# Chthi/Ofighters

Measured on AMD Instinct MI355X. Metric: arena-steps/sec (env.step+obs+policy fwd) at 4096 arenas, 1/2/4/8 MI355X, higher is better.
Workload: dtype f32; 1 GPU; 4096 arenas x 8 ships per GPU, random-bot actions + step + 2D obs rasterise (u8 maps) + bi-head policy forward for 8 ship(s)/arena, trunk shared per arena (BASELINE configs[3]); arenas_per_gpu=4096, ships=8, laser_cap=512, episode_ticks=200, parallelism=arena-sharded x1, RCCL all-reduce of episodic scores only, laser_overflow=0, last_episode_score_sum=71103, last_episode_arenas=4096

## Files before the change

include/ofx.h:

```cpp
#ifndef OFX_H
#define OFX_H

#include <stddef.h>
#include <stdint.h>

#ifdef __cplusplus
extern "C" {
#endif

#define OFX_VERSION 1

enum {
  OFX_OK = 0,
  OFX_ERR_INVALID = -1,
  OFX_ERR_NO_DEVICE = -2,
  OFX_ERR_HIP = -3,
  OFX_ERR_STATE = -4,
  OFX_ERR_OVERFLOW = -5
};

typedef struct ofx_config {
  int32_t n_arenas;
  int32_t n_ships;
  int32_t laser_cap;
// ... 121 lines not shown
  int32_t n_tensors;
} ofx_policy_desc;
int ofx_policy_layout(const ofx_handle *h, ofx_policy_desc *desc_host);
int ofx_policy_forward(ofx_handle *h, const float *weights, const uint8_t *ship_mask,
                       float *act_values, int32_t *iaction, int32_t *ipointer,
                       float *heatmap);
int ofx_policy_pin_weights(ofx_handle *h, const float *weights);
#define OFX_OPT_TRUNK_PLAIN 1
#define OFX_OPT_FRAMES_REF  2
#define OFX_OPT_TRUNK_FUSE  4
#define OFX_OPT_BILINEAR_LEGACY 3
#define OFX_OPT_POLICY_BF16 5
#define OFX_OPT_FIT_PLAIN 6
#define OFX_OPT_TRUNK_SPARSE 7
int ofx_policy_trunk_stats(ofx_handle *h, int64_t *counts_host);
int ofx_set_option(ofx_handle *h, int32_t option, int32_t value);
int ofx_policy_explore(ofx_handle *h, double epsilon, uint64_t seed, uint32_t tick, int32_t collecting,
                       const uint8_t *ship_mask, int32_t *iaction, int32_t *ipointer);
int ofx_policy_actions(ofx_handle *h, const int32_t *iaction, const int32_t *ipointer,
                       const uint8_t *ship_mask, ofx_action *actions);

typedef struct ofx_transition {
  int32_t tick_prev, tick_next;
  int32_t frame_prev, frame_next;
  int32_t ship;
  int32_t iaction, px, py;
  int32_t reward;
  int32_t done;
  float head_prev[8], head_next[8];
} ofx_transition;
// ... 39 lines not shown
```

ofighters_amd/_native.py:

```python
import ctypes as C
import os

_HERE = os.path.dirname(os.path.abspath(__file__))
LIB_PATH = os.path.join(_HERE, "libofx.so")

OFX_OK = 0
OFX_ERR_INVALID = -1
OFX_ERR_NO_DEVICE = -2
OFX_ERR_HIP = -3
OFX_ERR_STATE = -4
OFX_ERR_OVERFLOW = -5

BOT_IDLE, BOT_RANDOM, BOT_TURRET, BOT_RUNNER, BOT_THRUST, BOT_SHOOT = range(6)
BEHAVIOURS = {None: BOT_IDLE, "idle": BOT_IDLE, "random": BOT_RANDOM, "turret": BOT_TURRET,
              "runner": BOT_RUNNER, "thrust": BOT_THRUST, "shoot": BOT_SHOOT}

(F_SHIP_X, F_SHIP_Y, F_SHIP_PX, F_SHIP_PY, F_SHIP_ALIVE, F_REWARD, F_SCORE, F_N_LASERS, F_LASER_X, F_LASER_Y,
 F_LASER_OWNER, F_LASER_DEAD, F_KILLER, F_TIME, F_LAST_SCORES, F_HULL, F_LASER_DX, F_LASER_DY,
 F_OBS_REWARD) = range(19)

MAP_U8, MAP_F32, MAP_F64, MAP_BITS = range(4)
OPT_TRUNK_PLAIN, OPT_FRAMES_REF, OPT_BILINEAR_LEGACY, OPT_TRUNK_FUSE, OPT_POLICY_BF16, OPT_FIT_PLAIN, OPT_TRUNK_SPARSE = 1, 2, 3, 4, 5, 6, 7


# ... 85 lines not shown
    "ofx_replay_capture": (_i, [_vp, _u32, _vp, _vp, _vp]),
    "ofx_agents_first_done": (_i, [_vp, _vp, _vp, C.POINTER(C.c_int32)]),
    "ofx_replay_count": (_i, [_vp, _vp, _vp]),
    "ofx_replay_rows_host": (_i, [_vp, C.c_int32, _vp, _vp]),
    "ofx_replay_frame_host": (_i, [_vp, C.c_int32, C.c_int32, _vp, _vp]),
    "ofx_replay_sample": (_i, [_vp, _u64, _u32, C.c_int32, _vp, _vp]),
    "ofx_replay_gather": (_i, [_vp, _vp, C.c_int32, _vp, _vp, _vp]),
    "ofx_replay_gather_valid": (_i, [_vp, _vp, _vp, C.c_int32, C.c_int32, C.c_int32, _vp, _vp, _vp, _vp]),
    "ofx_timer_start": (_i, [_vp]),
    "ofx_timer_stop": (_i, [_vp, C.POINTER(C.c_float)]),
    "ofx_event_record": (_i, [_vp, C.c_int32]),
    "ofx_policy_profile": (_i, [_vp, C.c_int32]),
    "ofx_policy_pin_weights": (_i, [_vp, _vp]),
    "ofx_set_option": (_i, [_vp, C.c_int32, C.c_int32]),
    "ofx_policy_trunk_stats": (_i, [_vp, C.POINTER(C.c_int64)]),
    "ofx_event_elapsed": (_i, [_vp, C.c_int32, C.c_int32, C.POINTER(C.c_float)]),
}

_LIB = None


def lib():
    global _LIB
    if _LIB is None:
        if not os.path.exists(LIB_PATH):
            raise ImportError(
                "ofighters_amd: %s is missing - build it with `make -C ofighters_amd/csrc` "
                "(there is no CPU fallback)" % LIB_PATH)
        L = C.CDLL(LIB_PATH)
        for name, (res, args) in SIGNATURES.items():
# ... 21 lines not shown
```

ofighters_amd/csrc/ofx_api.hip:

```cpp
#include <math.h>
#include <stdarg.h>
#include <stdlib.h>
#include <string.h>

#include <new>

#include "ofx_internal.h"

static thread_local char g_err[512] = "";

void ofx_set_error(const char *fmt, ...) {
  va_list ap;
  va_start(ap, fmt);
  vsnprintf(g_err, sizeof(g_err), fmt, ap);
  va_end(ap);
}

extern "C" const char *ofx_last_error(void) { return g_err; }
extern "C" int ofx_version(void) { return OFX_VERSION; }

extern "C" int ofx_device_count(void) {
  int n = 0;
  if (hipGetDeviceCount(&n) != hipSuccess) return 0;
  return n;
// ... 95 lines not shown
  h->cfg = *cfg;
  h->hit_thresh = sqrt_le_threshold((double)(cfg->laser_radius + cfg->ship_radius));
  const size_t NM = (size_t)cfg->n_arenas * cfg->n_ships, NL = (size_t)cfg->n_arenas * cfg->laser_cap,
               N = (size_t)cfg->n_arenas;
  ofx_state &s = h->st;
#define A(field, count) if ((rc = dev_alloc_zero(&s.field, count))) { ofx_destroy(h); return rc; }
  A(ship_x, NM) A(ship_y, NM) A(ship_px, NM) A(ship_py, NM) A(hull, NM)
  A(reward, NM) A(score, NM) A(obs_reward, NM) A(last_score, NM)
  A(alive, NM) A(killer, NM)
  A(time, N) A(n_lasers, N)
  A(laser_x, NL) A(laser_y, NL) A(laser_dx, NL) A(laser_dy, NL)
  A(laser_owner, NL) A(laser_dead, NL)
  A(overflow, 1) A(episode_sums, (size_t)cfg->n_ships + 1)
#undef A
  if ((rc = dev_alloc_zero(&h->bot_behaviours, (size_t)cfg->n_ships))) { ofx_destroy(h); return rc; }
  h->n_cus = 256;
  { int v = 0; if (hipDeviceGetAttribute(&v, hipDeviceAttributeMultiprocessorCount, cfg->device) == hipSuccess && v > 0) h->n_cus = v; }
  hipError_t e = hipStreamCreateWithFlags(&h->stream, hipStreamNonBlocking);
  if (e != hipSuccess) { ofx_set_error("hipStreamCreate: %s", hipGetErrorString(e)); ofx_destroy(h); return OFX_ERR_HIP; }
  h->own_stream = true;
  h->prof_base = -1;
  e = hipDeviceSynchronize();
  if (e != hipSuccess) { ofx_set_error("hipDeviceSynchronize: %s", hipGetErrorString(e)); ofx_destroy(h); return OFX_ERR_HIP; }
  *out = h;
  return OFX_OK;
}

extern "C" int ofx_destroy(ofx_handle *h) {
  if (!h) return OFX_OK;
  (void)hipSetDevice(h->cfg.device);
// ... 531 lines not shown
```

ofighters_amd/csrc/ofx_policy.hip:

```cpp
#include <stdlib.h>
#include <string.h>
#include <type_traits>
#include <utility>

#include "ofx_internal.h"
#include "ofx_head.h"
#include "ofx_diag.h"
#include "ofx_lowp.h"

#define PS 400

typedef float f32x4 __attribute__((ext_vector_type(4)));
typedef float f32x2 __attribute__((ext_vector_type(2)));
typedef float f32x16 __attribute__((ext_vector_type(16)));

static const int kTrunkCin[4] = {2, 8, 8, 8};
static const int kUpCin[4] = {1, 2, 4, 8};
static const int kUpCout[4] = {2, 4, 8, 1};

static int policy_layout(int32_t *offset, int32_t *count) {
  int n = 0, off = 0;
#define T(c) do { offset[n] = off; count[n] = (c); off += (c); n++; } while (0)
  for (int i = 0; i < 4; i++) { T(9 * kTrunkCin[i] * 8); T(8); T(8); T(8); T(8); T(8); }
  T(5008 * 100); T(100);
// ... 192 lines not shown

struct ConvParams {
  const float *in;
  const unsigned *bits[2];
  size_t bits_stride;
  const float *w, *b;
  float *out;
  const uint8_t *mask;
  const float *wbm;
  int H, W;
  int tiles_x, tiles;
  int legacy;
  int images;
  const int32_t *live;
  unsigned long long *stat;
};

template <int CIN, int COUT, int TH, int TW, int MODE, bool POOL, bool OUT_HWC>
__global__ __launch_bounds__(((TH / 2) * (TW / 2) + 63) / 64 * 64) void k_conv(ConvParams p) {
  constexpr int NT = (TH / 2) * (TW / 2);
  constexpr int NTB = (NT + 63) / 64 * 64;
  constexpr int TWP = TW + 2;
  __shared__ __align__(16) float tile[CIN][TH + 2][TWP];
  const int img = blockIdx.x / p.tiles, t = blockIdx.x - img * p.tiles;
  if (p.mask && !p.mask[img]) return;
  const int ty0 = (t / p.tiles_x) * TH, tx0 = (t % p.tiles_x) * TW;
  const int tid = threadIdx.x;
  const int H = p.H, W = p.W;

  constexpr int TOTAL = CIN * (TH + 2) * TWP;
// ... 470 lines not shown
          d0 = __builtin_amdgcn_mfma_f32_16x16x4f32(a0[aof(j)], bw[j], d0, 0, 0, 0);
          d1 = __builtin_amdgcn_mfma_f32_16x16x4f32(a1[aof(j)], bw[j], d1, 0, 0, 0);
        }
        finish(d0, T);
        finish(d1, T1);
      } else {
        f32x4 d0 = binit;
#pragma unroll
        for (int j = 0; j < NK; j++) d0 = __builtin_amdgcn_mfma_f32_16x16x4f32(a0[aof(j)], bw[j], d0, 0, 0, 0);
        finish(d0, T);
      }
    }
  }
}

template <int WD, int RP, int LS, int PLS, int LP>
__device__ __forceinline__ void ts_gemm_phase_sparse(const float *abase, const float (&bw)[LP ? 1 : 24], const lp_x4 (&bwb)[6],
                                                     const f32x4 binit, int wv, int lane,
                                                     int n16, int kq, int r, float *orow, const unsigned *nz, float k2,
                                                     bool top, bool bottom, unsigned &n_exec, unsigned &n_all,
                                                     unsigned long long *dbg = nullptr) {
#if OFX_TRUNK_STAMPS
  unsigned long long g_last = __builtin_amdgcn_s_memtime();
#define TSG_STAMP(i) do { const unsigned long long t_ = __builtin_amdgcn_s_memtime(); dbg[i] += t_ - g_last; g_last = t_; } while (0)
#else
#define TSG_STAMP(i) do { } while (0)
#endif
  constexpr int NK = 24, NPX = RP * WD, NT = (NPX + 15) / 16;
  auto aof = [&](int j) -> int { return (4 * (j & 1)) * PLS + ((j >> 1) / 3) * LS + ((j >> 1) % 3); };
  int toff[6];
#pragma unroll
  for (int J = 0; J < 6; J++) {
    const int tap = 2 * J + (kq >> 1);
    toff[J] = (4 * (kq & 1) - kq) * PLS + (tap / 3) * LS + tap % 3;
  }
  auto mm1 = [&](const float *a0, f32x4 &d0) {
    if constexpr (LP != 0) {
#pragma unroll
      for (int J = 0; J < 6; J++) {
        const float *q0 = a0 + toff[J];
        d0 = lp_mfma16<LP ? LP : 1>(lp_pk4<LP ? LP : 1>(q0[0], q0[PLS], q0[2 * PLS], q0[3 * PLS]), bwb[J], d0);
      }
    } else {
// ... 48 lines not shown
        any |= (rw[0] & m0) | (rw[1] & m1);
      }
      run = any != 0u;
    }
    run_mask = __builtin_amdgcn_ballot_w64(run);
  }
  auto store_const = [&](int T) {
    const int P = 16 * T + 4 * kq, rp = P / WD, x = P - rp * WD;
    if (r == 0) *reinterpret_cast<float2 *>(orow + rp * (WD / 2) + (x >> 1)) = make_float2(k2, k2);
  };
  auto run1 = [&](int T0) {
    f32x4 d0 = binit;
    mm1(a_of_tile(T0), d0);
    finish(d0, T0);
  };
#pragma unroll 1
  for (int T = wv; T < NT; T += 16)
    if (!((run_mask >> T) & 1ull)) store_const(T);
  if (wv == 0) { n_all += (unsigned)NT; n_exec += (unsigned)__builtin_popcountll(run_mask); }
  TSG_STAMP(0);
  unsigned long long m = run_mask;
  for (int i = 0; i < wv && m; i++) m &= m - 1;
#pragma unroll 1
  while (m) {
    const int T0 = __builtin_ctzll(m);
    unsigned long long m2 = m;
    for (int i = 0; i < 16 && m2; i++) m2 &= m2 - 1;
    if (m2) {
      const int T1 = __builtin_ctzll(m2);
      f32x4 d0 = binit, d1 = binit;
      mm2(a_of_tile(T0), a_of_tile(T1), d0, d1);
      finish(d0, T0);
      finish(d1, T1);
// ... 37 lines not shown
    const float *a0 = a_of_tile(T), *a1 = a_of_tile(two ? T1 : T);
    f32x4 d0 = binit, d1 = binit;
#pragma unroll
    for (int J = 0; J < 6; J++) {
      const float *q0 = a0 + toff[J], *q1 = a1 + toff[J];
      const lp_x4 A0 = lp_pk4<LP>(q0[0], q0[PLS], q0[2 * PLS], q0[3 * PLS]);
      const lp_x4 A1 = lp_pk4<LP>(q1[0], q1[PLS], q1[2 * PLS], q1[3 * PLS]);
      d0 = lp_mfma16<LP>(A0, bwb[J], d0);
      d1 = lp_mfma16<LP>(A1, bwb[J], d1);
    }
    finish(d0, T);
    if (two) finish(d1, T1);
  }
}

constexpr int F12_TH = 10, F12_LS = 216, F12_ROWS = F12_TH + 2;
constexpr int F12_PLS = (F12_ROWS * F12_LS + 63) / 64 * 64 + 16;
constexpr int F12_WR = 14, F12_BR = 2 * (F12_TH + 1) + 2;
constexpr int F12_THREADS = 1024;
static_assert(F12_PLS % 64 == 16 && F12_PLS % 4 == 0 && F12_LS % 4 == 0, "tile layout");
static_assert(2 * F12_BR * F12_WR <= F12_THREADS, "one staged word per thread");
static_assert((F12_TH + 1) * 100 <= 2 * F12_THREADS && F12_TH * 100 <= F12_THREADS, "pixel pairs per step");

template <int LP, bool SPARSE = false>
__global__ __launch_bounds__(F12_THREADS) void k_trunk12(ConvParams p, const float *lut) {
  constexpr bool BF16 = LP != 0;
  constexpr int W = PS, H = PS, H1 = PS / 2, H2 = PS / 4, LS = F12_LS, PLS = F12_PLS, NK = 24;
  __shared__ __align__(16) float slut[2 * 512 * 8];
  __shared__ __align__(16) float tile[8 * F12_PLS];
  __shared__ unsigned rows[2][2][F12_BR][F12_WR];
  __shared__ __align__(16) float halo[2][8][2][F12_LS];
  __shared__ unsigned nz[SPARSE ? 2 : 1][F12_ROWS][8];
  __shared__ __align__(16) float k1s[8], k2s[8];
  __shared__ float wbs[(SPARSE && !BF16) ? 24 * 64 : 1];
  unsigned n_exec = 0, n_all = 0, t_exec = 0, t_all = 0;
#if OFX_TRUNK_STAMPS
  unsigned long long st_a = 0, st_b = 0, st_last = __builtin_amdgcn_s_memtime(), st_begin = st_last, st_g[3] = {0, 0, 0};
#define T12_STAMP(acc) do { const unsigned long long t_ = __builtin_amdgcn_s_memtime(); acc += t_ - st_last; st_last = t_; } while (0)
#else
#define T12_STAMP(acc) do { } while (0)
#endif
  const int tid = threadIdx.x, lane = tid & 63;
  const int wv = __builtin_amdgcn_readfirstlane(tid >> 6);
  const int n16 = lane & 15, kq = lane >> 4, co = n16 >> 1, r = n16 & 1;

  auto bits_fetch = [&](int img, int pa, int pb) -> unsigned {
    const int nrows = 2 * (pb - pa) + 2;
    unsigned out = 0u;
    if (tid < 2 * nrows * F12_WR) {
// ... 16 lines not shown
  };
  auto bits_commit = [&](int buf, int pa, int pb, unsigned word) {
    const int nrows = 2 * (pb - pa) + 2;
    if (tid < 2 * nrows * F12_WR) {
      const int w = tid % F12_WR, rr = (tid / F12_WR) % nrows, ci = tid / (F12_WR * nrows);
      rows[buf][ci][rr][w] = word;
    }
  };

  for (int e = tid; e < 2 * 512 * 8 / 4; e += F12_THREADS)
    reinterpret_cast<f32x4 *>(slut)[e] = reinterpret_cast<const f32x4 *>(lut)[e];
  for (int e = tid; e < 8 * PLS / 4; e += F12_THREADS) reinterpret_cast<f32x4 *>(tile)[e] = f32x4{0.f, 0.f, 0.f, 0.f};
  for (int e = tid; e < 2 * 8 * 2 * LS / 4; e += F12_THREADS) reinterpret_cast<f32x4 *>(&halo[0][0][0][0])[e] = f32x4{0.f, 0.f, 0.f, 0.f};
  float bw[(BF16 || SPARSE) ? 1 : NK];
  lp_x4 bwb[6];
  if constexpr (BF16) ts_bw_lp<LP ? LP : 1>(p.wbm, n16, kq, bwb);
  else if constexpr (SPARSE) {
    for (int e = tid; e < NK * 64; e += F12_THREADS) wbs[e] = p.wbm[e];
  } else {
#pragma unroll
    for (int j = 0; j < NK; j++) bw[j] = p.wbm[j * 64 + lane];
  }
  const float bias = p.b[co];
  const f32x4 binit = {bias, bias, bias, bias};
  const float *abase = &tile[kq * PLS + 3];
  if constexpr (SPARSE) {
    __syncthreads();
    if (tid < 8) k1s[tid] = fmaxf(slut[tid] + slut[512 * 8 + tid], 0.f);
    for (int e = tid; e < 2 * F12_ROWS * 8; e += F12_THREADS) (&nz[0][0][0])[e] = 0u;
    __syncthreads();
    for (int e = tid; e < 8 * PLS; e += F12_THREADS) tile[e] = k1s[min(e / PLS, 7)];
    __syncthreads();
    if (wv == 0) {
      const float *a0 = abase + 2 * LS + 16 + n16;
      f32x4 d0 = binit;
      if constexpr (BF16) {
#pragma unroll
        for (int J = 0; J < 6; J++) {
          const int tap = 2 * J + (kq >> 1);
          const float *q0 = a0 + (4 * (kq & 1) - kq) * PLS + (tap / 3) * LS + tap % 3;
          d0 = lp_mfma16<LP ? LP : 1>(lp_pk4<LP ? LP : 1>(q0[0], q0[PLS], q0[2 * PLS], q0[3 * PLS]), bwb[J], d0);
        }
      } else {
        auto aof = [&](int j) -> int { return (4 * (j & 1)) * PLS + ((j >> 1) / 3) * LS + ((j >> 1) % 3); };
#pragma unroll
        for (int j = 0; j < NK; j++) d0 = __builtin_amdgcn_mfma_f32_16x16x4f32(a0[aof(j)], wbs[(BF16 ? 0 : j) * 64 + lane], d0, 0, 0, 0);
      }
      float q0 = max_raw(max_raw(d0[0], 0.f), d0[1]);
      q0 = max_raw(q0, __builtin_bit_cast(float, __builtin_amdgcn_mov_dpp(__builtin_bit_cast(int, q0), 0xB1, 0xF, 0xF, true)));
      if (r == 0 && kq == 0) k2s[co] = q0;
    }
    __syncthreads();
    for (int e = tid; e < 8 * PLS / 4; e += F12_THREADS) reinterpret_cast<f32x4 *>(tile)[e] = f32x4{0.f, 0.f, 0.f, 0.f};
  }
  bits_commit(0, 0, F12_TH + 1, bits_fetch((int)blockIdx.x, 0, F12_TH + 1));
  unsigned w_ahead = 0u;
  if constexpr (SPARSE) { if ((int)blockIdx.x < p.images) w_ahead = bits_fetch((int)blockIdx.x, F12_TH + 1, 2 * F12_TH + 1); }
  __syncthreads();
  const float k2 = SPARSE ? k2s[co] : 0.f;

#pragma unroll 1
  for (int img = (int)blockIdx.x; img < p.images; img += (int)gridDim.x)
#pragma unroll 1
  for (int step = 0; step < H1 / F12_TH; step++) {
    const int R0 = step * F12_TH;
    const int pa = step ? R0 + 1 : 0, pb = min(R0 + F12_TH + 1, H1);
    const int buf = step & 1;
// ... 75 lines not shown
    }
    __syncthreads();

    T12_STAMP(st_a);
    if constexpr (!SPARSE) { if (more) nextw = bits_fetch(nimg, na, nb); }
    if constexpr (SPARSE) {
      if (more) bits_commit(buf ^ 1, na, nb, w_ahead);
      int i2 = nimg, s2 = last ? 0 : step + 1;
      if (++s2 == H1 / F12_TH) { s2 = 0; i2 += (int)gridDim.x; }
      const int r2 = s2 * F12_TH;
      w_ahead = i2 < p.images ? bits_fetch(i2, s2 ? r2 + 1 : 0, min(r2 + F12_TH + 1, H1)) : 0u;
    }

    if constexpr (SPARSE) {
      float bwl[BF16 ? 1 : NK];
      if constexpr (!BF16) {
        int zoff;
        asm volatile("s_mov_b32 %0, 0" : "=s"(zoff));
#pragma unroll
        for (int j = 0; j < NK; j++) bwl[j] = wbs[j * 64 + lane + zoff];
      }
      ts_gemm_phase_sparse<200, F12_TH / 2, F12_LS, F12_PLS, LP>(abase, bwl, bwb, binit, wv, lane, n16, kq, r,
                                                                  p.out + (((size_t)img * 8 + co) * H2 + (R0 >> 1)) * H2,
                                                                  &nz[buf][0][0], k2, step == 0, last, n_exec, n_all
#if OFX_TRUNK_STAMPS
                                                                  , st_g
#endif
                                                                  );
      for (int e = tid; e < F12_ROWS * 8; e += F12_THREADS) (&nz[buf ^ 1][0][0])[e] = 0u;
    } else if constexpr (BF16)
      ts_gemm_phase_bf16<200, F12_TH / 2, F12_LS, F12_PLS, LP ? LP : 1>(abase, bwb, binit, wv, n16, kq, r,
                                                            p.out + (((size_t)img * 8 + co) * H2 + (R0 >> 1)) * H2);
    else
      ts_gemm_phase<200, F12_TH / 2, F12_LS, F12_PLS>(abase, bw, binit, wv, n16, kq, r,
                                                       p.out + (((size_t)img * 8 + co) * H2 + (R0 >> 1)) * H2);
    if constexpr (!SPARSE) { if (more) bits_commit(buf ^ 1, na, nb, nextw); }
    __syncthreads();
  }
  if constexpr (SPARSE) {
// ... 6 lines not shown
#else
    if (p.stat && lane == 0) {
      atomicAdd(&p.stat[0], (unsigned long long)n_exec); atomicAdd(&p.stat[1], (unsigned long long)n_all);
      atomicAdd(&p.stat[2], (unsigned long long)t_exec); atomicAdd(&p.stat[3], (unsigned long long)t_all);
    }
#endif
  }
}

constexpr int C3_W = 100, C3_TH = 20, C3_LS = 108, C3_ROWS = C3_TH + 2, C3_F4 = C3_LS / 4;
constexpr int C3_PLS = (C3_ROWS * C3_LS + 63) / 64 * 64 + 16;
constexpr int C3_PF4 = C3_ROWS * C3_F4, C3_NI = (C3_PF4 + 63) / 64;
static_assert(C3_PLS % 64 == 16 && C3_W % C3_TH == 0 && C3_W / 4 + 2 == C3_F4 && 64 * C3_NI * 4 <= C3_PLS + 64 * 4, "tile layout");
static_assert(2 * 8 * C3_PLS * 4 <= 160 * 1024, "two tiles in LDS");

template <int LP>
__global__ __launch_bounds__(F12_THREADS) void k_conv3_stream(ConvParams p, const float *zero16) {
  constexpr bool BF16 = LP != 0;
  constexpr int W = C3_W, H = C3_W, H2 = C3_W / 2, PLS = C3_PLS, NK = 24, STEPS = H / C3_TH;
  __shared__ __align__(16) float tiles[2][8 * C3_PLS];
  const int tid = threadIdx.x, lane = tid & 63;
  const int wv = __builtin_amdgcn_readfirstlane(tid >> 6);
  const int n16 = lane & 15, kq = lane >> 4, co = n16 >> 1, r = n16 & 1;

  auto stage = [&](int buf, int img, int R0) {
#pragma unroll 1
    for (int i = wv; i < 8 * C3_NI; i += F12_THREADS / 64) {
      const int ci = i / C3_NI, k = i - ci * C3_NI;
      const int q = 64 * k + lane;
      if (q < C3_PF4) {
        const int row = q / C3_F4, c4 = q - row * C3_F4, gy = R0 - 1 + row;
        const float *src = zero16;
        if (c4 >= 1 && c4 <= W / 4 && gy >= 0 && gy < H) src = p.in + (((size_t)img * 8 + ci) * H + gy) * W + 4 * (c4 - 1);
        __builtin_amdgcn_global_load_lds((const __attribute__((address_space(1))) void *)src,
                                         (__attribute__((address_space(3))) void *)&tiles[buf][ci * PLS + 256 * k], 16, 0, 0);
      }
    }
  };

  float bw[BF16 ? 1 : NK];
  lp_x4 bwb[6];
  if constexpr (BF16) ts_bw_lp<LP ? LP : 1>(p.wbm, n16, kq, bwb);
  else {
#pragma unroll
    for (int j = 0; j < NK; j++) bw[j] = p.wbm[j * 64 + lane];
  }
  const float bias = p.b[co];
  const f32x4 binit = {bias, bias, bias, bias};
  if ((int)blockIdx.x < p.images) stage(0, (int)blockIdx.x, 0);
  __builtin_amdgcn_s_waitcnt(0x0F70);
  __syncthreads();
  int buf = 0;
#pragma unroll 1
  for (int img = (int)blockIdx.x; img < p.images; img += (int)gridDim.x)
#pragma unroll 1
  for (int step = 0; step < STEPS; step++) {
    const int R0 = step * C3_TH;
    const bool last = step + 1 == STEPS;
    const int nimg = last ? img + (int)gridDim.x : img;
    if (nimg < p.images) stage(buf ^ 1, nimg, last ? 0 : R0 + C3_TH);
    if constexpr (BF16)
      ts_gemm_phase_bf16<W, C3_TH / 2, C3_LS, C3_PLS, LP ? LP : 1>(&tiles[buf][kq * PLS + 3], bwb, binit, wv, n16, kq, r,
                                                      p.out + (((size_t)img * 8 + co) * H2 + (R0 >> 1)) * H2);
    else
      ts_gemm_phase<W, C3_TH / 2, C3_LS, C3_PLS>(&tiles[buf][kq * PLS + 3], bw, binit, wv, n16, kq, r,
                                                 p.out + (((size_t)img * 8 + co) * H2 + (R0 >> 1)) * H2);
    __builtin_amdgcn_s_waitcnt(0x0F70);
    __syncthreads();
    buf ^= 1;
  }
}


__global__ __launch_bounds__(256) void k_gemm_f32(const float *A, int lda, const float *B, int ldb, const float *bias,
                                                  float *C, int ldc, int M, int N, int K, int relu, const int32_t *live) {
  const int lane = threadIdx.x & 63, wv = threadIdx.x >> 6;
  const int tiles_n = (N + 31) / 32;
  const int tile = blockIdx.x * 4 + wv;
  if (live) M = live[0];
  if (tile >= ((M + 31) / 32) * tiles_n) return;
  const int m0 = (tile / tiles_n) * 32, n0 = (tile % tiles_n) * 32;
  const int r0 = m0 + (lane & 31), c = n0 + (lane & 31), kh = lane >> 5;
  const bool rv = r0 < M, cv = c < N;
  const int r = live ? live[1 + (rv ? r0 : 0)] : r0;
// ... 141 lines not shown
  if (s >= S || (mask && !mask[s])) return;
  ofx_action a;
  a.valid = st.alive[s] ? 1 : 0;
  a.shoot = iaction[s] == 0;
  a.thrust = iaction[s] == 1;
  a.px = ipointer[2 * s];
  a.py = ipointer[2 * s + 1];
  a._pad = 0;
  out[s] = a;
}

struct PolicyWs {
  float *p1, *p2, *p3, *p4, *g1, *d1, *u0, *up1, *u2fr, *vfr, *c4;
  unsigned long long *best;
  int32_t *iaction, *ipointer, *live;
};

static size_t al(size_t b) { return (b + 255) & ~(size_t)255; }
constexpr int kDense1Chunks = 25;

static bool trunk_fused(const ofx_handle *h, size_t N) {
  if (h->opt_trunk_plain) return false;
  return h->opt_trunk_fuse == 1 || (h->opt_trunk_fuse == 0 && N >= 4 * (size_t)h->n_cus);
}

static int policy_workspace(ofx_handle *h, PolicyWs *ws, size_t N, size_t S) {
  size_t f2, f3, f4;
  ofx_head_frame_bytes(S, &f2, &f3, &f4);
  const size_t sz[] = {trunk_fused(h, N) ? 0 : al(4ull * N * 8 * 200 * 200), al(4ull * N * 8 * 100 * 100), al(4ull * N * 8 * 50 * 50),
                       al(4ull * N * 5000),          al(4ull * N * 100 * kDense1Chunks), al(4ull * S * 100),
                       al(4ull * S * 625),           al(4ull * S * 2 * 50 * 50),   al(f2), al(f3), al(f4),
                       al(8ull * S),                 al(4ull * S),                 al(8ull * S),
                       al(4ull * (S + 1))};
  size_t total = 0;
  for (size_t b : sz) total += b;
  int rc = ofx_ensure_scratch(h, total);
  if (rc) return rc;
  char *base = (char *)h->scratch;
  void **dst[] = {(void **)&ws->p1,   (void **)&ws->p2,   (void **)&ws->p3,      (void **)&ws->p4,      (void **)&ws->g1,
                  (void **)&ws->d1,   (void **)&ws->u0,   (void **)&ws->up1,     (void **)&ws->u2fr,    (void **)&ws->vfr,
                  (void **)&ws->c4,   (void **)&ws->best, (void **)&ws->iaction, (void **)&ws->ipointer,
                  (void **)&ws->live};
  for (size_t i = 0; i < sizeof(sz) / sizeof(sz[0]); i++) { *dst[i] = base; base += sz[i]; }
  return OFX_OK;
}

template <int CIN, int COUT, int TH, int TW, int MODE, bool POOL, bool OUT_HWC>
static int launch_conv(ofx_handle *h, ConvParams p, int images, int H) {
  p.H = H; p.W = H;
  p.tiles_x = H / TW;
  p.tiles = p.tiles_x * (H / TH);
  constexpr int NTB = ((TH / 2) * (TW / 2) + 63) / 64 * 64;
  hipLaunchKernelGGL((k_conv<CIN, COUT, TH, TW, MODE, POOL, OUT_HWC>), dim3((unsigned)(images * p.tiles)), dim3(NTB), 0,
                     h->stream, p);
  OFX_HIP(hipGetLastError());
  return OFX_OK;
}
// ... 55 lines not shown
  if (!h) { ofx_set_error("ofx_policy_pin_weights: null handle"); return OFX_ERR_INVALID; }
  OFX_HIP(hipSetDevice(h->cfg.device));
  h->prep_pinned = nullptr;
  if (!weights) return OFX_OK;
  int rc = policy_prepare(h, weights, &h->prep);
  if (rc) return rc;
  h->prep_pinned = weights;
  return OFX_OK;
}

int ofx_policy_weights_updated(ofx_handle *h, const float *weights) {
  if (h->prep_pinned && h->prep_pinned == weights) return policy_prepare(h, weights, &h->prep);
  return OFX_OK;
}

extern "C" int ofx_policy_trunk_stats(ofx_handle *h, int64_t *counts_host) {
  if (!h || !counts_host) { ofx_set_error("ofx_policy_trunk_stats: null argument"); return OFX_ERR_INVALID; }
  for (int i = 0; i < 4; i++) counts_host[i] = 0;
  if (!h->trunk_stat) return OFX_OK;
  OFX_HIP(hipSetDevice(h->cfg.device));
  OFX_HIP(hipMemcpyAsync(counts_host, h->trunk_stat, 4 * sizeof(unsigned long long), hipMemcpyDeviceToHost, h->stream));
  OFX_HIP(hipMemsetAsync(h->trunk_stat, 0, 4 * sizeof(unsigned long long), h->stream));
  OFX_HIP(hipStreamSynchronize(h->stream));
  return OFX_OK;
}

extern "C" int ofx_set_option(ofx_handle *h, int32_t option, int32_t value) {
  if (!h) { ofx_set_error("ofx_set_option: null handle"); return OFX_ERR_INVALID; }
  switch (option) {
    case OFX_OPT_TRUNK_PLAIN: h->opt_trunk_plain = value != 0; return OFX_OK;
    case OFX_OPT_TRUNK_FUSE:
      if (value < 0 || value > 2) { ofx_set_error("ofx_set_option: OFX_OPT_TRUNK_FUSE takes 0 (auto), 1 (always), 2 (never)"); return OFX_ERR_INVALID; }
      h->opt_trunk_fuse = value; return OFX_OK;
    case OFX_OPT_FRAMES_REF: h->opt_frames_ref = value != 0; return OFX_OK;
    case OFX_OPT_TRUNK_SPARSE:
      if (value && !h->trunk_stat) {
        OFX_HIP(hipSetDevice(h->cfg.device));
        OFX_HIP(hipMalloc((void **)&h->trunk_stat, 4 * sizeof(unsigned long long)));
        OFX_HIP(hipMemsetAsync(h->trunk_stat, 0, 4 * sizeof(unsigned long long), h->stream));
      }
      h->opt_trunk_sparse = value != 0; return OFX_OK;
    case OFX_OPT_FIT_PLAIN: h->opt_fit_plain = value != 0; return OFX_OK;
    case OFX_OPT_POLICY_BF16:
      if (value < 0 || value > 2) { ofx_set_error("ofx_set_option: OFX_OPT_POLICY_BF16 takes 0 (fp32), 1 (bf16 operands), 2 (fp16 operands)"); return OFX_ERR_INVALID; }
      h->opt_policy_lowp = value; return OFX_OK;
    case OFX_OPT_BILINEAR_LEGACY:
      if (h->opt_bilinear_legacy == (value != 0)) return OFX_OK;
      h->opt_bilinear_legacy = value != 0;
      OFX_HIP(hipSetDevice(h->cfg.device));
      return h->prep_pinned ? policy_prepare(h, h->prep_pinned, &h->prep) : OFX_OK;
    default: ofx_set_error("ofx_set_option: unknown option %d", option); return OFX_ERR_INVALID;
  }
}

// ... 10 lines not shown
  const PrepLayout L = prep_layout();

  const bool pinned = h->prep && h->prep_pinned == weights;
  if (!pinned && (rc = policy_prepare(h, weights, &h->prep_tmp))) return rc;
  const float *prep = pinned ? h->prep : h->prep_tmp;

  ConvParams cp;
  memset(&cp, 0, sizeof(cp));
  cp.bits[0] = bits0;
  cp.bits[1] = bits1;
  cp.bits_stride = bits_stride;
  cp.w = prep + L.tw[0]; cp.b = prep + L.tb[0]; cp.out = ws.p1;
  const int lowp = vec8 == nullptr ? h->opt_policy_lowp : 0;
  const bool plain = h->opt_trunk_plain;
  const bool fused12 = trunk_fused(h, (size_t)N);
  if (plain) rc = launch_conv<2, 8, 10, 100, 1, true, false>(h, cp, N, 400);
  else if (fused12) {
    cp.out = ws.p2; cp.b = prep + L.tb[1]; cp.wbm = prep + L.wbm[0]; cp.images = N;
    const dim3 g12((unsigned)(N < h->n_cus ? N : h->n_cus));
    const bool sparse = h->opt_trunk_sparse || vec8 != nullptr;
    cp.stat = h->opt_trunk_sparse ? h->trunk_stat : nullptr;
    const float *lut1 = prep + L.lut1;
#define T12(LP_) do { if (sparse) hipLaunchKernelGGL((k_trunk12<LP_, true>), g12, dim3(F12_THREADS), 0, h->stream, cp, lut1); \
                      else hipLaunchKernelGGL((k_trunk12<LP_, false>), g12, dim3(F12_THREADS), 0, h->stream, cp, lut1); } while (0)
    if (lowp == 1) T12(1); else if (lowp == 2) T12(2); else T12(0);
#undef T12
    OFX_HIP(hipGetLastError());
  } else {
    cp.H = 400; cp.W = 400;
    hipLaunchKernelGGL(k_conv1_lut<40>, dim3((unsigned)(N * (400 / 40))), dim3(256), 0, h->stream, cp,
                       (const float *)(prep + L.lut1));
    OFX_HIP(hipGetLastError());
  }
  if (rc) return rc;
  cp.in = ws.p1; cp.w = prep + L.tw[1]; cp.b = prep + L.tb[1]; cp.out = ws.p2; cp.wbm = prep + L.wbm[0];
  if (plain) rc = launch_conv<8, 8, 10, 100, 0, true, false>(h, cp, N, 200);
  else if (!fused12) rc = launch_convm<8, 2, 13, 0, false, 1>(h, cp, N, 200);
  if (rc) return rc;
  cp.in = ws.p2; cp.w = prep + L.tw[2]; cp.b = prep + L.tb[2]; cp.out = ws.p3; cp.wbm = prep + L.wbm[1];
  if (plain) rc = launch_conv<8, 8, 10, 100, 0, true, false>(h, cp, N, 100);
  else if (fused12) {
    cp.images = N;
    const dim3 g3((unsigned)(N < h->n_cus ? N : h->n_cus));
    if (lowp == 1) hipLaunchKernelGGL(k_conv3_stream<1>, g3, dim3(F12_THREADS), 0, h->stream, cp, (const float *)(prep + L.zero16));
    else if (lowp == 2) hipLaunchKernelGGL(k_conv3_stream<2>, g3, dim3(F12_THREADS), 0, h->stream, cp, (const float *)(prep + L.zero16));
    else hipLaunchKernelGGL(k_conv3_stream<0>, g3, dim3(F12_THREADS), 0, h->stream, cp, (const float *)(prep + L.zero16));
    OFX_HIP(hipGetLastError());
  } else rc = launch_convm<8, 4, 7, 0, false, 1>(h, cp, N, 100);
  if (rc) return rc;
  cp.in = ws.p3; cp.w = prep + L.tw[3]; cp.b = prep + L.tb[3]; cp.out = ws.p4; cp.wbm = prep + L.wbm[2];
  if (plain) rc = launch_conv<8, 8, 10, 50, 0, true, true>(h, cp, N, 50);
  else if (lowp == 1 && fused12) rc = launch_convm<8, 10, 4, 0, true, 1, 1>(h, cp, N, 50);
  else if (lowp == 2 && fused12) rc = launch_convm<8, 10, 4, 0, true, 1, 2>(h, cp, N, 50);
  else rc = launch_convm<8, 10, 4, 0, true, 1>(h, cp, N, 50);
  if (rc) return rc;

  const float *k1 = weights + off[t_d1];
  {
    const int tiles = ((N + 31) / 32) * 4, jobs = tiles * kDense1Chunks;
    hipLaunchKernelGGL(k_gemm_f32_splitk, dim3((jobs + 3) / 4), dim3(256), 0, h->stream, ws.p4, 5000, k1 + 8 * 100, 100,
                       ws.g1, N, 100, 5000 / kDense1Chunks, tiles, jobs);
// ... 225 lines not shown
```

ofighters_amd/engine.py:

```python
import ctypes as C

import numpy as np

from . import _native as nat

_FIELD_DTYPE = {
    nat.F_SHIP_X: np.int32, nat.F_SHIP_Y: np.int32, nat.F_SHIP_PX: np.int32, nat.F_SHIP_PY: np.int32,
    nat.F_SHIP_ALIVE: np.uint8, nat.F_REWARD: np.int32, nat.F_SCORE: np.int32, nat.F_N_LASERS: np.int32,
    nat.F_LASER_X: np.float64, nat.F_LASER_Y: np.float64, nat.F_LASER_OWNER: np.uint8,
    nat.F_LASER_DEAD: np.uint8, nat.F_KILLER: np.int16, nat.F_TIME: np.int32, nat.F_LAST_SCORES: np.int32,
    nat.F_HULL: np.int32, nat.F_LASER_DX: np.float64, nat.F_LASER_DY: np.float64, nat.F_OBS_REWARD: np.int32,
}
_MAP_DTYPE = {nat.MAP_U8: np.uint8, nat.MAP_F32: np.float32, nat.MAP_F64: np.float64, nat.MAP_BITS: np.uint8}

ACTION_DTYPE = np.dtype([("px", np.int32), ("py", np.int32), ("shoot", np.uint8), ("thrust", np.uint8),
                         ("valid", np.uint8), ("_pad", np.uint8)])
assert ACTION_DTYPE.itemsize == C.sizeof(nat.OfxAction) == 12


class DeviceBuffer:

    def __init__(self, nbytes):
        self.nbytes = int(nbytes)
        p = C.c_void_p()
# ... 262 lines not shown
                       heat_ptr=None):
        nat.check(nat.lib().ofx_policy_forward(self._h, weights_ptr, ship_mask_ptr, act_ptr, iaction_ptr,
                                               ipointer_ptr, heat_ptr))

    def policy_pin_weights(self, weights_ptr):
        nat.check(nat.lib().ofx_policy_pin_weights(self._h, weights_ptr))

    def set_option(self, option, value):
        nat.check(nat.lib().ofx_set_option(self._h, int(option), int(value)))

    def policy_trunk_stats(self):
        v = (C.c_int64 * 4)()
        nat.check(nat.lib().ofx_policy_trunk_stats(self._h, v))
        return tuple(int(x) for x in v)

    def policy_actions(self, out_ptr=None, iaction_ptr=None, ipointer_ptr=None, ship_mask_ptr=None):
        out_ptr = out_ptr or self._actions.ptr
        nat.check(nat.lib().ofx_policy_actions(self._h, iaction_ptr, ipointer_ptr, ship_mask_ptr, out_ptr))
        return out_ptr

    def policy_forward_host(self, weights, ship_mask=None, want_heat=False):
        S = self.N * self.M
        w = np.ascontiguousarray(weights, np.float32)
        dw = DeviceBuffer(w.nbytes).upload(w)
        dm = None
        if ship_mask is not None:
            m = np.ascontiguousarray(ship_mask, np.uint8).reshape(S)
            dm = DeviceBuffer(m.nbytes).upload(m)
        da, di, dp = DeviceBuffer(8 * S), DeviceBuffer(4 * S), DeviceBuffer(8 * S)
        dh = DeviceBuffer(4 * S * self.W * self.H) if want_heat else None
# ... 149 lines not shown
```

Before: 216,600 arena-steps/s.

## Propagate constant-tile map from fused trunk to skip constant conv3 tiles

The fused conv1/2 trunk kernel now records, per pooled row, a bitmask of 8-pixel groups whose output is a known constant, and stores the constant per channel. Conv3 becomes a sparse variant that loads these masks a few steps ahead, redirects constant inputs to the constant vector, and skips MFMA work for tiles whose whole receptive field is constant. Sparse trunk mode is also turned on by default at handle creation. The cost is extra map traffic, more LDS and extra branching, and correctness now depends on the constant-value bookkeeping holding across both kernels.

```diff
diff --git a/include/ofx.h b/include/ofx.h
--- a/include/ofx.h
+++ b/include/ofx.h
@@ -159,6 +159,7 @@
 #define OFX_OPT_FIT_PLAIN 6
 #define OFX_OPT_TRUNK_SPARSE 7
 int ofx_policy_trunk_stats(ofx_handle *h, int64_t *counts_host);
+int ofx_policy_conv3_stats(ofx_handle *h, int64_t *counts_host);
 int ofx_set_option(ofx_handle *h, int32_t option, int32_t value);
 int ofx_policy_explore(ofx_handle *h, double epsilon, uint64_t seed, uint32_t tick, int32_t collecting,
                        const uint8_t *ship_mask, int32_t *iaction, int32_t *ipointer);
diff --git a/ofighters_amd/_native.py b/ofighters_amd/_native.py
--- a/ofighters_amd/_native.py
+++ b/ofighters_amd/_native.py
@@ -123,6 +123,7 @@
     "ofx_policy_pin_weights": (_i, [_vp, _vp]),
     "ofx_set_option": (_i, [_vp, C.c_int32, C.c_int32]),
     "ofx_policy_trunk_stats": (_i, [_vp, C.POINTER(C.c_int64)]),
+    "ofx_policy_conv3_stats": (_i, [_vp, C.POINTER(C.c_int64)]),
     "ofx_event_elapsed": (_i, [_vp, C.c_int32, C.c_int32, C.POINTER(C.c_float)]),
 }
 
diff --git a/ofighters_amd/csrc/ofx_api.hip b/ofighters_amd/csrc/ofx_api.hip
--- a/ofighters_amd/csrc/ofx_api.hip
+++ b/ofighters_amd/csrc/ofx_api.hip
@@ -133,6 +133,7 @@
   A(overflow, 1) A(episode_sums, (size_t)cfg->n_ships + 1)
 #undef A
   if ((rc = dev_alloc_zero(&h->bot_behaviours, (size_t)cfg->n_ships))) { ofx_destroy(h); return rc; }
+  h->opt_trunk_sparse = true;
   h->n_cus = 256;
   { int v = 0; if (hipDeviceGetAttribute(&v, hipDeviceAttributeMultiprocessorCount, cfg->device) == hipSuccess && v > 0) h->n_cus = v; }
   hipError_t e = hipStreamCreateWithFlags(&h->stream, hipStreamNonBlocking);
diff --git a/ofighters_amd/csrc/ofx_policy.hip b/ofighters_amd/csrc/ofx_policy.hip
--- a/ofighters_amd/csrc/ofx_policy.hip
+++ b/ofighters_amd/csrc/ofx_policy.hip
@@ -230,6 +230,8 @@
   int images;
   const int32_t *live;
   unsigned long long *stat;
+  unsigned *cmap;
+  float *kc;
 };
 
 template <int CIN, int COUT, int TH, int TW, int MODE, bool POOL, bool OUT_HWC>
@@ -730,19 +732,21 @@
   }
 }
 
-template <int WD, int RP, int LS, int PLS, int LP>
+template <int WD, int RP, int LS, int PLS, int LP, bool MAP = false>
 __device__ __forceinline__ void ts_gemm_phase_sparse(const float *abase, const float (&bw)[LP ? 1 : 24], const lp_x4 (&bwb)[6],
                                                      const f32x4 binit, int wv, int lane,
                                                      int n16, int kq, int r, float *orow, const unsigned *nz, float k2,
                                                      bool top, bool bottom, unsigned &n_exec, unsigned &n_all,
-                                                     unsigned long long *dbg = nullptr) {
+                                                     unsigned *cmap = nullptr, unsigned long long *dbg = nullptr) {
 #if OFX_TRUNK_STAMPS
   unsigned long long g_last = __builtin_amdgcn_s_memtime();
-#define TSG_STAMP(i) do { const unsigned long long t_ = __builtin_amdgcn_s_memtime(); dbg[i] += t_ - g_last; g_last = t_; } while (0)
+#define TSG_STAMP(i) do { if (dbg) { const unsigned long long t_ = __builtin_amdgcn_s_memtime(); dbg[i] += t_ - g_last; g_last = t_; } } while (0)
 #else
 #define TSG_STAMP(i) do { } while (0)
 #endif
   constexpr int NK = 24, NPX = RP * WD, NT = (NPX + 15) / 16;
+  static_assert(NT <= 64 && WD % 4 == 0, "one lane per M-tile of the step");
+  static_assert(!MAP || (WD % 8 == 0 && WD / 8 <= 32), "one map word per pooled row: whole float4 of 8-pixel groups");
   auto aof = [&](int j) -> int { return (4 * (j & 1)) * PLS + ((j >> 1) / 3) * LS + ((j >> 1) % 3); };
   int toff[6];
 #pragma unroll
@@ -821,9 +825,19 @@
     mm1(a_of_tile(T0), d0);
     finish(d0, T0);
   };
+  if constexpr (MAP) {
+    if (wv == 0 && lane < RP) {
+      unsigned word = 0u;
 #pragma unroll 1
-  for (int T = wv; T < NT; T += 16)
-    if (!((run_mask >> T) & 1ull)) store_const(T);
+      for (int j = 0; j < WD / 8; j++)
+        if (!((run_mask >> ((lane * WD + 8 * j) >> 4)) & 1ull)) word |= 1u << j;
+      cmap[lane] = word;
+    }
+  } else {
+#pragma unroll 1
+    for (int T = wv; T < NT; T += 16)
+      if (!((run_mask >> T) & 1ull)) store_const(T);
+  }
   if (wv == 0) { n_all += (unsigned)NT; n_exec += (unsigned)__builtin_popcountll(run_mask); }
   TSG_STAMP(0);
   unsigned long long m = run_mask;
@@ -891,6 +905,25 @@
   }
 }
 
+template <int LS, int PLS, int LP, class BW>
+__device__ __forceinline__ float ts_const_tile(const float *a0, BW bwj, const lp_x4 (&bwb)[6], const f32x4 binit, int kq) {
+  f32x4 d0 = binit;
+  if constexpr (LP != 0) {
+#pragma unroll
+    for (int J = 0; J < 6; J++) {
+      const int tap = 2 * J + (kq >> 1);
+      const float *q0 = a0 + (4 * (kq & 1) - kq) * PLS + (tap / 3) * LS + tap % 3;
+      d0 = lp_mfma16<LP ? LP : 1>(lp_pk4<LP ? LP : 1>(q0[0], q0[PLS], q0[2 * PLS], q0[3 * PLS]), bwb[J], d0);
+    }
+  } else {
+    auto aof = [&](int j) -> int { return (4 * (j & 1)) * PLS + ((j >> 1) / 3) * LS + ((j >> 1) % 3); };
+#pragma unroll
+    for (int j = 0; j < 24; j++) d0 = __builtin_amdgcn_mfma_f32_16x16x4f32(a0[aof(j)], bwj(j), d0, 0, 0, 0);
+  }
+  float q0 = max_raw(max_raw(d0[0], 0.f), d0[1]);
+  return max_raw(q0, __builtin_bit_cast(float, __builtin_amdgcn_mov_dpp(__builtin_bit_cast(int, q0), 0xB1, 0xF, 0xF, true)));
+}
+
 constexpr int F12_TH = 10, F12_LS = 216, F12_ROWS = F12_TH + 2;
 constexpr int F12_PLS = (F12_ROWS * F12_LS + 63) / 64 * 64 + 16;
 constexpr int F12_WR = 14, F12_BR = 2 * (F12_TH + 1) + 2;
@@ -910,6 +943,7 @@
   __shared__ unsigned nz[SPARSE ? 2 : 1][F12_ROWS][8];
   __shared__ __align__(16) float k1s[8], k2s[8];
   __shared__ float wbs[(SPARSE && !BF16) ? 24 * 64 : 1];
+  __shared__ lp_x4 wbl[(SPARSE && BF16) ? 6 * 64 : 1];
   unsigned n_exec = 0, n_all = 0, t_exec = 0, t_all = 0;
 #if OFX_TRUNK_STAMPS
   unsigned long long st_a = 0, st_b = 0, st_last = __builtin_amdgcn_s_memtime(), st_begin = st_last, st_g[3] = {0, 0, 0};
@@ -956,8 +990,15 @@
   for (int e = tid; e < 2 * 8 * 2 * LS / 4; e += F12_THREADS) reinterpret_cast<f32x4 *>(&halo[0][0][0][0])[e] = f32x4{0.f, 0.f, 0.f, 0.f};
   float bw[(BF16 || SPARSE) ? 1 : NK];
   lp_x4 bwb[6];
-  if constexpr (BF16) ts_bw_lp<LP ? LP : 1>(p.wbm, n16, kq, bwb);
-  else if constexpr (SPARSE) {
+  if constexpr (BF16) {
+    ts_bw_lp<LP ? LP : 1>(p.wbm, n16, kq, bwb);
+    if constexpr (SPARSE) {
+      if (wv == 0) {
+#pragma unroll
+        for (int J = 0; J < 6; J++) wbl[J * 64 + lane] = bwb[J];
+      }
+    }
+  } else if constexpr (SPARSE) {
     for (int e = tid; e < NK * 64; e += F12_THREADS) wbs[e] = p.wbm[e];
   } else {
 #pragma unroll
@@ -974,25 +1015,12 @@
     for (int e = tid; e < 8 * PLS; e += F12_THREADS) tile[e] = k1s[min(e / PLS, 7)];
     __syncthreads();
     if (wv == 0) {
-      const float *a0 = abase + 2 * LS + 16 + n16;
-      f32x4 d0 = binit;
-      if constexpr (BF16) {
-#pragma unroll
-        for (int J = 0; J < 6; J++) {
-          const int tap = 2 * J + (kq >> 1);
-          const float *q0 = a0 + (4 * (kq & 1) - kq) * PLS + (tap / 3) * LS + tap % 3;
-          d0 = lp_mfma16<LP ? LP : 1>(lp_pk4<LP ? LP : 1>(q0[0], q0[PLS], q0[2 * PLS], q0[3 * PLS]), bwb[J], d0);
-        }
-      } else {
-        auto aof = [&](int j) -> int { return (4 * (j & 1)) * PLS + ((j >> 1) / 3) * LS + ((j >> 1) % 3); };
-#pragma unroll
-        for (int j = 0; j < NK; j++) d0 = __builtin_amdgcn_mfma_f32_16x16x4f32(a0[aof(j)], wbs[(BF16 ? 0 : j) * 64 + lane], d0, 0, 0, 0);
-      }
-      float q0 = max_raw(max_raw(d0[0], 0.f), d0[1]);
-      q0 = max_raw(q0, __builtin_bit_cast(float, __builtin_amdgcn_mov_dpp(__builtin_bit_cast(int, q0), 0xB1, 0xF, 0xF, true)));
+      const float q0 = ts_const_tile<LS, PLS, LP>(abase + 2 * LS + 16 + n16, [&](int j) { return wbs[(BF16 ? 0 : j) * 64 + lane]; },
+                                                  bwb, binit, kq);
       if (r == 0 && kq == 0) k2s[co] = q0;
     }
     __syncthreads();
+    if (blockIdx.x == 0 && tid < 32) p.kc[tid] = k2s[tid >> 2];
     for (int e = tid; e < 8 * PLS / 4; e += F12_THREADS) reinterpret_cast<f32x4 *>(tile)[e] = f32x4{0.f, 0.f, 0.f, 0.f};
   }
   bits_commit(0, 0, F12_TH + 1, bits_fetch((int)blockIdx.x, 0, F12_TH + 1));
@@ -1098,15 +1126,20 @@
 
     if constexpr (SPARSE) {
       float bwl[BF16 ? 1 : NK];
+      lp_x4 bwbl[6];
+      int zoff;
+      asm volatile("s_mov_b32 %0, 0" : "=s"(zoff));
       if constexpr (!BF16) {
-        int zoff;
-        asm volatile("s_mov_b32 %0, 0" : "=s"(zoff));
 #pragma unroll
         for (int j = 0; j < NK; j++) bwl[j] = wbs[j * 64 + lane + zoff];
-      }
-      ts_gemm_phase_sparse<200, F12_TH / 2, F12_LS, F12_PLS, LP>(abase, bwl, bwb, binit, wv, lane, n16, kq, r,
+      } else {
+#pragma unroll
+        for (int J = 0; J < 6; J++) bwbl[J] = wbl[J * 64 + lane + zoff];
+      }
+      ts_gemm_phase_sparse<200, F12_TH / 2, F12_LS, F12_PLS, LP, true>(abase, bwl, bwbl, binit, wv, lane, n16, kq, r,
                                                                   p.out + (((size_t)img * 8 + co) * H2 + (R0 >> 1)) * H2,
-                                                                  &nz[buf][0][0], k2, step == 0, last, n_exec, n_all
+                                                                  &nz[buf][0][0], k2, step == 0, last, n_exec, n_all,
+                                                                  p.cmap + (size_t)img * H2 + (R0 >> 1)
 #if OFX_TRUNK_STAMPS
                                                                   , st_g
 #endif
@@ -1143,26 +1176,58 @@
 static_assert(C3_PLS % 64 == 16 && C3_W % C3_TH == 0 && C3_W / 4 + 2 == C3_F4 && 64 * C3_NI * 4 <= C3_PLS + 64 * 4, "tile layout");
 static_assert(2 * 8 * C3_PLS * 4 <= 160 * 1024, "two tiles in LDS");
 
-template <int LP>
+template <int LP, bool SPARSE = false>
 __global__ __launch_bounds__(F12_THREADS) void k_conv3_stream(ConvParams p, const float *zero16) {
   constexpr bool BF16 = LP != 0;
   constexpr int W = C3_W, H = C3_W, H2 = C3_W / 2, PLS = C3_PLS, NK = 24, STEPS = H / C3_TH;
   __shared__ __align__(16) float tiles[2][8 * C3_PLS];
+  __shared__ unsigned nz[SPARSE ? 3 : 1][SPARSE ? C3_ROWS : 1][8];
+  __shared__ float k3s[8];
+  unsigned n_exec = 0, n_all = 0;
   const int tid = threadIdx.x, lane = tid & 63;
   const int wv = __builtin_amdgcn_readfirstlane(tid >> 6);
   const int n16 = lane & 15, kq = lane >> 4, co = n16 >> 1, r = n16 & 1;
 
-  auto stage = [&](int buf, int img, int R0) {
-#pragma unroll 1
-    for (int i = wv; i < 8 * C3_NI; i += F12_THREADS / 64) {
+  static_assert(8 * C3_NI % (F12_THREADS / 64) == 0, "the same number of stage loads in every wave");
+  auto stage = [&](int buf, int img, int R0, const unsigned *marks) {
+    auto load = [&](int i) {
       const int ci = i / C3_NI, k = i - ci * C3_NI;
       const int q = 64 * k + lane;
       if (q < C3_PF4) {
         const int row = q / C3_F4, c4 = q - row * C3_F4, gy = R0 - 1 + row;
         const float *src = zero16;
-        if (c4 >= 1 && c4 <= W / 4 && gy >= 0 && gy < H) src = p.in + (((size_t)img * 8 + ci) * H + gy) * W + 4 * (c4 - 1);
+        if (c4 >= 1 && c4 <= W / 4 && gy >= 0 && gy < H) {
+          src = p.in + (((size_t)img * 8 + ci) * H + gy) * W + 4 * (c4 - 1);
+          if constexpr (SPARSE) {
+            const int x = 4 * (c4 - 1);
+            if (!((marks[row * 8 + (x >> 5)] >> (x & 31)) & 1u)) src = p.kc + 4 * ci;
+          }
+        }
         __builtin_amdgcn_global_load_lds((const __attribute__((address_space(1))) void *)src,
                                          (__attribute__((address_space(3))) void *)&tiles[buf][ci * PLS + 256 * k], 16, 0, 0);
+      }
+    };
+    if constexpr (SPARSE) {
+#pragma unroll
+      for (int it = 0; it < 8 * C3_NI / (F12_THREADS / 64); it++) load(wv + it * (F12_THREADS / 64));
+    } else {
+#pragma unroll 1
+      for (int i = wv; i < 8 * C3_NI; i += F12_THREADS / 64) load(i);
+    }
+  };
+  auto map_fetch = [&](int img, int step) -> unsigned {
+    const int gy = step * C3_TH - 1 + lane;
+    return (lane < C3_ROWS && img < p.images && gy >= 0 && gy < H) ? p.cmap[(size_t)img * H + gy] : 0u;
+  };
+  auto marks_commit = [&](int slot, unsigned word) {
+    if (lane < C3_ROWS) {
+#pragma unroll
+      for (int k = 0; k < 8; k++) {
+        unsigned m = 0xFFFFFFFFu;
+#pragma unroll
+        for (int i = 0; i < 8; i++)
+          if (8 * k + i < W / 4 && ((word >> (8 * k + i)) & 1u)) m &= ~(0xFu << (4 * i));
+        nz[slot][lane][k] = m;
       }
     }
   };
@@ -1176,10 +1241,23 @@
   }
   const float bias = p.b[co];
   const f32x4 binit = {bias, bias, bias, bias};
-  if ((int)blockIdx.x < p.images) stage(0, (int)blockIdx.x, 0);
+  if constexpr (SPARSE) {
+    for (int e = tid; e < 8 * PLS; e += F12_THREADS) tiles[0][e] = p.kc[4 * min(e / PLS, 7)];
+    if (wv == 0) marks_commit(0, map_fetch((int)blockIdx.x, 0));
+    if (wv == 1) marks_commit(1, map_fetch((int)blockIdx.x, 1));
+    __syncthreads();
+    if (wv == 0) {
+      const float q0 = ts_const_tile<C3_LS, PLS, LP>(&tiles[0][kq * PLS + 3] + 2 * C3_LS + 16 + n16,
+                                                     [&](int j) { return bw[BF16 ? 0 : j]; }, bwb, binit, kq);
+      if (r == 0 && kq == 0) k3s[co] = q0;
+    }
+    __syncthreads();
+  }
+  if ((int)blockIdx.x < p.images) stage(0, (int)blockIdx.x, 0, &nz[0][0][0]);
   __builtin_amdgcn_s_waitcnt(0x0F70);
   __syncthreads();
-  int buf = 0;
+  const float k3 = SPARSE ? k3s[co] : 0.f;
+  int buf = 0, slot = 0;
 #pragma unroll 1
   for (int img = (int)blockIdx.x; img < p.images; img += (int)gridDim.x)
 #pragma unroll 1
@@ -1187,16 +1265,31 @@
     const int R0 = step * C3_TH;
     const bool last = step + 1 == STEPS;
     const int nimg = last ? img + (int)gridDim.x : img;
-    if (nimg < p.images) stage(buf ^ 1, nimg, last ? 0 : R0 + C3_TH);
-    if constexpr (BF16)
-      ts_gemm_phase_bf16<W, C3_TH / 2, C3_LS, C3_PLS, LP ? LP : 1>(&tiles[buf][kq * PLS + 3], bwb, binit, wv, n16, kq, r,
-                                                      p.out + (((size_t)img * 8 + co) * H2 + (R0 >> 1)) * H2);
+    const int slot1 = slot == 2 ? 0 : slot + 1, slot2 = slot1 == 2 ? 0 : slot1 + 1;
+    unsigned word2 = 0u;
+    if constexpr (SPARSE) {
+      if (wv == 15) {
+        const int s2 = step + 2 < STEPS ? step + 2 : step + 2 - STEPS;
+        word2 = map_fetch(step + 2 < STEPS ? img : img + (int)gridDim.x, s2);
+      }
+    }
+    if (nimg < p.images) stage(buf ^ 1, nimg, last ? 0 : R0 + C3_TH, &nz[SPARSE ? slot1 : 0][0][0]);
+    float *orow = p.out + (((size_t)img * 8 + co) * H2 + (R0 >> 1)) * H2;
+    if constexpr (SPARSE)
+      ts_gemm_phase_sparse<W, C3_TH / 2, C3_LS, C3_PLS, LP>(&tiles[buf][kq * PLS + 3], bw, bwb, binit, wv, lane, n16, kq, r,
+                                                            orow, &nz[slot][0][0], k3, step == 0, last, n_exec, n_all);
+    else if constexpr (BF16)
+      ts_gemm_phase_bf16<W, C3_TH / 2, C3_LS, C3_PLS, LP ? LP : 1>(&tiles[buf][kq * PLS + 3], bwb, binit, wv, n16, kq, r, orow);
     else
-      ts_gemm_phase<W, C3_TH / 2, C3_LS, C3_PLS>(&tiles[buf][kq * PLS + 3], bw, binit, wv, n16, kq, r,
-                                                 p.out + (((size_t)img * 8 + co) * H2 + (R0 >> 1)) * H2);
+      ts_gemm_phase<W, C3_TH / 2, C3_LS, C3_PLS>(&tiles[buf][kq * PLS + 3], bw, binit, wv, n16, kq, r, orow);
     __builtin_amdgcn_s_waitcnt(0x0F70);
+    if constexpr (SPARSE) { if (wv == 15) marks_commit(slot2, word2); }
     __syncthreads();
     buf ^= 1;
+    slot = slot1;
+  }
+  if constexpr (SPARSE) {
+    if (p.stat && lane == 0 && wv == 0) { atomicAdd(&p.stat[0], (unsigned long long)n_exec); atomicAdd(&p.stat[1], (unsigned long long)n_all); }
   }
 }
 
@@ -1368,6 +1461,8 @@
   float *p1, *p2, *p3, *p4, *g1, *d1, *u0, *up1, *u2fr, *vfr, *c4;
   unsigned long long *best;
   int32_t *iaction, *ipointer, *live;
+  unsigned *cmap;
+  float *kc;
 };
 
 static size_t al(size_t b) { return (b + 255) & ~(size_t)255; }
@@ -1385,7 +1480,7 @@
                        al(4ull * N * 5000),          al(4ull * N * 100 * kDense1Chunks), al(4ull * S * 100),
                        al(4ull * S * 625),           al(4ull * S * 2 * 50 * 50),   al(f2), al(f3), al(f4),
                        al(8ull * S),                 al(4ull * S),                 al(8ull * S),
-                       al(4ull * (S + 1))};
+                       al(4ull * (S + 1)),           al(4ull * N * 100),           al(4ull * 32)};
   size_t total = 0;
   for (size_t b : sz) total += b;
   int rc = ofx_ensure_scratch(h, total);
@@ -1394,7 +1489,7 @@
   void **dst[] = {(void **)&ws->p1,   (void **)&ws->p2,   (void **)&ws->p3,      (void **)&ws->p4,      (void **)&ws->g1,
                   (void **)&ws->d1,   (void **)&ws->u0,   (void **)&ws->up1,     (void **)&ws->u2fr,    (void **)&ws->vfr,
                   (void **)&ws->c4,   (void **)&ws->best, (void **)&ws->iaction, (void **)&ws->ipointer,
-                  (void **)&ws->live};
+                  (void **)&ws->live, (void **)&ws->cmap, (void **)&ws->kc};
   for (size_t i = 0; i < sizeof(sz) / sizeof(sz[0]); i++) { *dst[i] = base; base += sz[i]; }
   return OFX_OK;
 }
@@ -1480,6 +1575,8 @@
   return OFX_OK;
 }
 
+constexpr int kTrunkStats = 6;
+
 extern "C" int ofx_policy_trunk_stats(ofx_handle *h, int64_t *counts_host) {
   if (!h || !counts_host) { ofx_set_error("ofx_policy_trunk_stats: null argument"); return OFX_ERR_INVALID; }
   for (int i = 0; i < 4; i++) counts_host[i] = 0;
@@ -1487,6 +1584,17 @@
   OFX_HIP(hipSetDevice(h->cfg.device));
   OFX_HIP(hipMemcpyAsync(counts_host, h->trunk_stat, 4 * sizeof(unsigned long long), hipMemcpyDeviceToHost, h->stream));
   OFX_HIP(hipMemsetAsync(h->trunk_stat, 0, 4 * sizeof(unsigned long long), h->stream));
+  OFX_HIP(hipStreamSynchronize(h->stream));
+  return OFX_OK;
+}
+
+extern "C" int ofx_policy_conv3_stats(ofx_handle *h, int64_t *counts_host) {
+  if (!h || !counts_host) { ofx_set_error("ofx_policy_conv3_stats: null argument"); return OFX_ERR_INVALID; }
+  for (int i = 0; i < 2; i++) counts_host[i] = 0;
+  if (!h->trunk_stat) return OFX_OK;
+  OFX_HIP(hipSetDevice(h->cfg.device));
+  OFX_HIP(hipMemcpyAsync(counts_host, h->trunk_stat + 4, 2 * sizeof(unsigned long long), hipMemcpyDeviceToHost, h->stream));
+  OFX_HIP(hipMemsetAsync(h->trunk_stat + 4, 0, 2 * sizeof(unsigned long long), h->stream));
   OFX_HIP(hipStreamSynchronize(h->stream));
   return OFX_OK;
 }
@@ -1502,8 +1610,8 @@
     case OFX_OPT_TRUNK_SPARSE:
       if (value && !h->trunk_stat) {
         OFX_HIP(hipSetDevice(h->cfg.device));
-        OFX_HIP(hipMalloc((void **)&h->trunk_stat, 4 * sizeof(unsigned long long)));
-        OFX_HIP(hipMemsetAsync(h->trunk_stat, 0, 4 * sizeof(unsigned long long), h->stream));
+        OFX_HIP(hipMalloc((void **)&h->trunk_stat, kTrunkStats * sizeof(unsigned long long)));
+        OFX_HIP(hipMemsetAsync(h->trunk_stat, 0, kTrunkStats * sizeof(unsigned long long), h->stream));
       }
       h->opt_trunk_sparse = value != 0; return OFX_OK;
     case OFX_OPT_FIT_PLAIN: h->opt_fit_plain = value != 0; return OFX_OK;
@@ -1544,12 +1652,13 @@
   const int lowp = vec8 == nullptr ? h->opt_policy_lowp : 0;
   const bool plain = h->opt_trunk_plain;
   const bool fused12 = trunk_fused(h, (size_t)N);
+  const bool sparse = fused12 && h->opt_trunk_sparse;
   if (plain) rc = launch_conv<2, 8, 10, 100, 1, true, false>(h, cp, N, 400);
   else if (fused12) {
     cp.out = ws.p2; cp.b = prep + L.tb[1]; cp.wbm = prep + L.wbm[0]; cp.images = N;
     const dim3 g12((unsigned)(N < h->n_cus ? N : h->n_cus));
-    const bool sparse = h->opt_trunk_sparse || vec8 != nullptr;
-    cp.stat = h->opt_trunk_sparse ? h->trunk_stat : nullptr;
+    cp.stat = sparse ? h->trunk_stat : nullptr;
+    cp.cmap = ws.cmap; cp.kc = ws.kc;
     const float *lut1 = prep + L.lut1;
 #define T12(LP_) do { if (sparse) hipLaunchKernelGGL((k_trunk12<LP_, true>), g12, dim3(F12_THREADS), 0, h->stream, cp, lut1); \
                       else hipLaunchKernelGGL((k_trunk12<LP_, false>), g12, dim3(F12_THREADS), 0, h->stream, cp, lut1); } while (0)
@@ -1571,10 +1680,13 @@
   if (plain) rc = launch_conv<8, 8, 10, 100, 0, true, false>(h, cp, N, 100);
   else if (fused12) {
     cp.images = N;
+    cp.stat = sparse && h->trunk_stat ? h->trunk_stat + 4 : nullptr;
     const dim3 g3((unsigned)(N < h->n_cus ? N : h->n_cus));
-    if (lowp == 1) hipLaunchKernelGGL(k_conv3_stream<1>, g3, dim3(F12_THREADS), 0, h->stream, cp, (const float *)(prep + L.zero16));
-    else if (lowp == 2) hipLaunchKernelGGL(k_conv3_stream<2>, g3, dim3(F12_THREADS), 0, h->stream, cp, (const float *)(prep + L.zero16));
-    else hipLaunchKernelGGL(k_conv3_stream<0>, g3, dim3(F12_THREADS), 0, h->stream, cp, (const float *)(prep + L.zero16));
+    const float *zero16 = prep + L.zero16;
+#define C3(LP_) do { if (sparse) hipLaunchKernelGGL((k_conv3_stream<LP_, true>), g3, dim3(F12_THREADS), 0, h->stream, cp, zero16); \
+                     else hipLaunchKernelGGL((k_conv3_stream<LP_, false>), g3, dim3(F12_THREADS), 0, h->stream, cp, zero16); } while (0)
+    if (lowp == 1) C3(1); else if (lowp == 2) C3(2); else C3(0);
+#undef C3
     OFX_HIP(hipGetLastError());
   } else rc = launch_convm<8, 4, 7, 0, false, 1>(h, cp, N, 100);
   if (rc) return rc;
diff --git a/ofighters_amd/engine.py b/ofighters_amd/engine.py
--- a/ofighters_amd/engine.py
+++ b/ofighters_amd/engine.py
@@ -300,6 +300,11 @@
         nat.check(nat.lib().ofx_policy_trunk_stats(self._h, v))
         return tuple(int(x) for x in v)
 
+    def policy_conv3_stats(self):
+        v = (C.c_int64 * 2)()
+        nat.check(nat.lib().ofx_policy_conv3_stats(self._h, v))
+        return tuple(int(x) for x in v)
+
     def policy_actions(self, out_ptr=None, iaction_ptr=None, ipointer_ptr=None, ship_mask_ptr=None):
         out_ptr = out_ptr or self._actions.ptr
         nat.check(nat.lib().ofx_policy_actions(self._h, iaction_ptr, ipointer_ptr, ship_mask_ptr, out_ptr))
```

Result: faster. 224,100 arena-steps/s, median of 6 (+3.4%).
